# G-Research/ahocorasick_rs

Hardware: NVIDIA H100
Metric: haystack_GB_per_s_scanned_find_matches_as_indexes (higher is better)
Workload: dtype u8

## Files before the change

### ahocorasick_rs_b200/csrc/scan_staged.cuh

```cuda
#pragma once
#include <type_traits>

#include "scan_core.cuh"

namespace acb {

#ifndef ACB_MAX_WARPS
#define ACB_MAX_WARPS 32
#endif
constexpr int kMaxWarps = ACB_MAX_WARPS;
#ifndef ACB_MAX_WARPS2
#define ACB_MAX_WARPS2 22
#endif
constexpr int kMaxWarps2 = ACB_MAX_WARPS2;
constexpr int kChunk = 64;
constexpr int kRow = kChunk;
constexpr int kStageBytes = 32 * kRow;
constexpr int kStageOffset = 256 + 128;
constexpr int kMetaBytes = 32 * 8;

struct FastTab {
    uint32_t cmap;
    uint32_t lo, maxc;
};

__device__ __forceinline__ uint32_t lds_tab(uint32_t addr) {
    uint32_t v;
    asm("ld.shared.u16 %0, [%1];\n" : "=r"(v) : "r"(addr));
    return v;
}
__device__ __forceinline__ uint32_t lds_tab_u8(uint32_t addr) {
    uint32_t v;
    asm("ld.shared.u8 %0, [%1];\n" : "=r"(v) : "r"(addr));
    return v;
}
__device__ __forceinline__ uint4 lds128(uint32_t addr) {
    uint4 v;
    asm volatile("ld.shared.v4.u32 {%0, %1, %2, %3}, [%4];\n" : "=r"(v.x), "=r"(v.y), "=r"(v.z), "=r"(v.w) : "r"(addr));
    return v;
}
__device__ __forceinline__ uint32_t lds8(uint32_t addr) {
    uint32_t v;
    asm volatile("ld.shared.u8 %0, [%1];\n" : "=r"(v) : "r"(addr));
    return v;
}
__device__ __forceinline__ uint32_t lds32(uint32_t addr) {
    uint32_t v;
    asm("ld.shared.u32 %0, [%1];\n" : "=r"(v) : "r"(addr));
    return v;
}
__device__ __forceinline__ uint2 lds64(uint32_t addr) {
    uint2 v;
    asm volatile("ld.shared.v2.u32 {%0, %1}, [%2];\n" : "=r"(v.x), "=r"(v.y) : "r"(addr));
    return v;
}
__device__ __forceinline__ void sts64(uint32_t addr, uint2 v) {
    asm volatile("st.shared.v2.u32 [%0], {%1, %2};\n" ::"r"(addr), "r"(v.x), "r"(v.y) : "memory");
}
__device__ __forceinline__ uint32_t row_unit(uint32_t row, uint32_t j) { return row ^ (j << 4); }
__device__ __forceinline__ uint32_t row_byte(uint32_t row, uint32_t p) { return (row ^ (p & 0x30u)) + (p & 15u); }

constexpr int kColAscii = 2;

template <int COLMODE, bool CLAMP = true>
__device__ __forceinline__ uint32_t fstep(uint32_t s, uint32_t b, const FastTab &f) {
    uint32_t col;
    if (COLMODE == kColRange)
        col = min(b - f.lo, f.maxc);
    else if (COLMODE == kColClass)
        col = lds_tab_u8(f.cmap + b);
    else
        col = CLAMP ? min(b, 127u) : b;
    uint32_t addr;
    asm("mad.lo.u32 %0, %1, 2, %2;\n" : "=r"(addr) : "r"(col), "r"(s));
    return lds_tab(addr);
}

template <uint32_t K>
__device__ __forceinline__ uint32_t fstep_dp(uint32_t s, uint32_t w) {
    uint32_t addr;
    asm("dp4a.u32.u32 %0, %1, %2, %3;\n" : "=r"(addr) : "r"(w), "r"(2u << (8 * K)), "r"(s));
    return lds_tab(addr);
}
__device__ __forceinline__ uint32_t clamp7f(uint32_t w) {
    const uint32_t hi = w & 0x80808080u;
    return (w | (hi - (hi >> 7))) & ~hi;
}

template <int COLMODE, bool CLAMP = true>
__device__ __forceinline__ uint32_t fstep4(uint32_t s, uint32_t w, const FastTab &f) {
    if (COLMODE == kColAscii && !CLAMP) {
        s = fstep_dp<0>(s, w);
        s = fstep_dp<1>(s, w);
        s = fstep_dp<2>(s, w);
        return fstep_dp<3>(s, w);
    }
    s = fstep<COLMODE, CLAMP>(s, __byte_perm(w, 0, 0x4440), f);
    s = fstep<COLMODE, CLAMP>(s, __byte_perm(w, 0, 0x4441), f);
    s = fstep<COLMODE, CLAMP>(s, __byte_perm(w, 0, 0x4442), f);
    s = fstep<COLMODE, CLAMP>(s, __byte_perm(w, 0, 0x4443), f);
    return s;
}

__device__ __forceinline__ uint32_t cont_bytes(uint32_t w) { return __popc(w & ~(w << 1) & 0x80808080u); }

__device__ __forceinline__ void cp_async16(uint32_t dst_smem, const void *src, uint32_t src_bytes) {
    asm volatile("cp.async.cg.shared.global.L2::128B [%0], [%1], 16, %2;\n" ::"r"(dst_smem), "l"(src), "r"(src_bytes) : "memory");
}
__device__ __forceinline__ void cp_async16_last(uint32_t dst_smem, const void *src, uint32_t src_bytes) {
    asm volatile(
        "{\n"
        ".reg .b64 pol;\n"
        "createpolicy.fractional.L2::evict_first.b64 pol, 1.0;\n"
        "cp.async.cg.shared.global.L2::cache_hint.L2::128B [%0], [%1], 16, %2, pol;\n"
        "}\n" ::"r"(dst_smem), "l"(src), "r"(src_bytes)
        : "memory");
}
__device__ __forceinline__ void cp_async_commit() { asm volatile("cp.async.commit_group;\n" ::: "memory"); }
__device__ __forceinline__ void cp_async_wait_all() { asm volatile("cp.async.wait_group 0;\n" ::: "memory"); }

__device__ __forceinline__ void mbar_init(uint32_t bar, uint32_t count) {
    asm volatile("mbarrier.init.shared::cta.b64 [%0], %1;\n" ::"r"(bar), "r"(count) : "memory");
    asm volatile("fence.mbarrier_init.release.cluster;\n" ::: "memory");
}
__device__ __forceinline__ void mbar_expect_tx(uint32_t bar, uint32_t bytes) {
    asm volatile("mbarrier.arrive.expect_tx.shared::cta.b64 _, [%0], %1;\n" ::"r"(bar), "r"(bytes) : "memory");
}
__device__ __forceinline__ void tma_bulk_g2s(uint32_t dst, const void *src, uint32_t bytes, uint32_t bar) {
    asm volatile("cp.async.bulk.shared::cluster.global.mbarrier::complete_tx::bytes [%0], [%1], %2, [%3];\n" ::"r"(dst),
                 "l"(src), "r"(bytes), "r"(bar)
                 : "memory");
}
__device__ __forceinline__ void mbar_wait(uint32_t bar, uint32_t parity) {
    asm volatile(
        "{\n"
        ".reg .pred p;\n"
        "WAIT_%=:\n"
        "mbarrier.try_wait.parity.shared::cta.b64 p, [%0], %1;\n"
        "@p bra DONE_%=;\n"
        "bra WAIT_%=;\n"
        "DONE_%=:\n"
        "}\n" ::"r"(bar),
        "r"(parity)
        : "memory");
}

struct DevHot {
    const uint16_t *table;
    const uint32_t *hot2full;
    const uint16_t *full2hot;
    uint32_t n_rows;
    const uint16_t *table128;
    uint32_t n_rows128;
};

enum PieceKind : uint32_t { kPieceWarm = 0, kPieceHead = 1, kPieceNormal = 2 };
struct LaneSeg {
    int64_t org;
    int64_t seg;
    uint32_t lo_rel, hi_rel;
    uint32_t h;
    uint32_t kind;
    uint32_t spec_state, head_count;
    uint32_t done;
    uint32_t far;
};

template <int MODE, bool CP>
__device__ __forceinline__ void advance_piece(PieceCtx &c, LaneSeg &L, const Batch &B, const Sink &out, const SegOut &seg_out) {
    bool finish_segment = false;
    if (L.kind == kPieceWarm) {
        const uint32_t he_rel = c.limit;
        const uint32_t piece_end = min(L.hi_rel, he_rel);
        if (c.at == L.lo_rel) {
            L.spec_state = c.state;
            L.kind = kPieceHead;
            c.stop = piece_end;
            c.emit_from = 0;
            c.cp_pos = c.at;
            c.cp_cont = 0;
            return;
        }
        L.spec_state = kSpecSkipped;
        L.kind = kPieceHead;
        c.at = piece_end;
        c.stop = piece_end;
        c.emit_from = 0;
        c.state = kRoot;
        c.have = 0;
        c.cp_pos = L.lo_rel;
        c.cp_cont = 0;
    }
    if (L.kind == kPieceHead) L.head_count = c.nemit;
    if (c.stop == c.limit) {
        int64_t h = (int64_t)L.h + 1;
        while (h < B.n_haystacks && __ldg(B.offsets + h + 1) == __ldg(B.offsets + h)) h++;
        const int64_t hi_pos = L.org + L.hi_rel;
        if (h < B.n_haystacks && __ldg(B.offsets + h) < hi_pos) {
            const int64_t hs = __ldg(B.offsets + h), he = __ldg(B.offsets + h + 1);
            L.h = (uint32_t)h;
            L.kind = kPieceNormal;
            c.at = (uint32_t)(hs - L.org);
// ... 53 lines not shown
    const uint32_t cmap_s = hot_s + hot_bytes;
    const uint32_t bar_s = cmap_s + 256;
    const uint32_t h2f_s = cmap_s + kStageOffset;
    const uint32_t stage_all_s = h2f_s + (((H + 1) * 4 + 127u) & ~127u);
    const uint32_t row_entries = COLMODE == kColAscii ? kAsciiCols : im.n_cols;
    const uint32_t row_bytes = row_entries * 2;
    const uint32_t trap_off = H * row_bytes;
    const uint32_t trap = hot_s + trap_off;
    const uint16_t *src_table = COLMODE == kColAscii ? hot_img.table128 : hot_img.table;
    uint8_t *cmap = smem + hot_bytes;
    int64_t *bounds = reinterpret_cast<int64_t *>(smem + hot_bytes + 256 + 16);

    const uint32_t n_entries = (H + 1) * row_entries;
    const uint32_t guard_entries = COLMODE == kColAscii ? kAsciiCols : 0;
    uint32_t *tab32 = reinterpret_cast<uint32_t *>(smem);
    const uint32_t bias2 = hot_s | (hot_s << 16);
    if (H == (COLMODE == kColAscii ? hot_img.n_rows128 : hot_img.n_rows)) {
        const uint32_t bytes = (n_entries * 2 + 15u) & ~15u;
        if (threadIdx.x == 0) {
            mbar_init(bar_s, 1);
            mbar_expect_tx(bar_s, bytes);
            tma_bulk_g2s(hot_s, src_table, bytes, bar_s);
            bounds[0] = __ldg(B.offsets);
            bounds[1] = __ldg(B.offsets + B.n_haystacks);
        }
        for (uint32_t i = threadIdx.x; i < 256; i += blockDim.x) cmap[i] = __ldg(im.colmap + i);
        __syncthreads();
        mbar_wait(bar_s, 0);
        for (uint32_t i = threadIdx.x; i < (n_entries + 1) / 2; i += blockDim.x) tab32[i] += bias2;
    } else {
        const uint32_t n = H * row_entries;
        const uint32_t *src32 = reinterpret_cast<const uint32_t *>(src_table);
        for (uint32_t i = threadIdx.x; i < (n + 1) / 2; i += blockDim.x) {
            const uint32_t v = __ldg(src32 + i);
            tab32[i] = (min(v & 0xffffu, trap_off) | (min(v >> 16, trap_off) << 16)) + bias2;
        }
        __syncthreads();
        uint16_t *h16 = reinterpret_cast<uint16_t *>(smem);
        for (uint32_t i = threadIdx.x; i < row_entries; i += blockDim.x) h16[n + i] = (uint16_t)trap;
        for (uint32_t i = threadIdx.x; i < 256; i += blockDim.x) cmap[i] = __ldg(im.colmap + i);
        if (threadIdx.x == 0) {
            bounds[0] = __ldg(B.offsets);
            bounds[1] = __ldg(B.offsets + B.n_haystacks);
        }
    }
    {
        uint16_t *h16 = reinterpret_cast<uint16_t *>(smem);
        for (uint32_t i = threadIdx.x; i < guard_entries; i += blockDim.x) h16[n_entries + i] = (uint16_t)trap;
        uint32_t *h2f = reinterpret_cast<uint32_t *>(smem + hot_bytes + kStageOffset);
        for (uint32_t i = threadIdx.x; i <= H; i += blockDim.x) h2f[i] = i < H ? __ldg(hot_img.hot2full + i) : kDead;
    }
    __syncthreads();
    if (blockIdx.x == 0 && threadIdx.x == 0) atomicAdd(trap_stats, (unsigned long long)((bounds[1] - bounds[0]) >> 4));

    HotMap hm;
    hm.full2hot = hot_img.full2hot;
    hm.hot_limit = H;
    FastTab ft;
    ft.cmap = cmap_s;
    ft.lo = im.col_lo;
    ft.maxc = im.n_cols - 1;
    auto row_of = [&](uint32_t addr) { return (addr - hot_s) / row_bytes; };
    auto state_of = [&](uint32_t addr) { return lds32(h2f_s + row_of(addr) * 4); };

    const uint32_t lane = threadIdx.x & 31, warp = threadIdx.x >> 5;
    constexpr uint32_t kRows = 32 * V;
    constexpr uint32_t kBufBytes = kRows * kRow;
    constexpr uint32_t kWarpMeta = kRows * 8;
    const uint32_t meta_s = stage_all_s + warp * kWarpMeta;
    const uint32_t stage_s = stage_all_s + (blockDim.x >> 5) * kWarpMeta + warp * 2 * kBufBytes;
    const uintptr_t gbase = reinterpret_cast<uintptr_t>(B.bytes + P.origin);
    const uint32_t cp_dst = stage_s + (lane >> 2) * kRow + (((lane & 3) ^ ((lane >> 3) & 3)) << 4);
    const uint32_t cp_meta = meta_s + (lane >> 2) * 8;
    const uint32_t row_s = stage_s + lane * kRow + (((lane >> 1) & 3) << 4);
    const uint32_t q = P.lane_stride;
    const uint32_t n_tasks = (uint32_t)(((uint64_t)P.n_segments + (uint64_t)kRows * q - 1) / ((uint64_t)kRows * q) * q);

    PieceCtx c_mem[V];
    LaneSeg L_mem[V];
    PieceCtx *c_ptr = c_mem;
    LaneSeg *L_ptr = L_mem;
    asm volatile("" : "+l"(c_ptr), "+l"(L_ptr));

    unsigned int claimed = 0;
    if (lane == 0) claimed = atomicAdd(task_counter, 1u);
    for (;;) {
        const unsigned int task = __shfl_sync(0xffffffffu, claimed, 0);
        if (task >= n_tasks) break;

        uint32_t pos[V], s[V], stop[V], cpd[V];
        uint32_t hi_rel[V], stop_head[V];
        bool done[V], warm[V];
        uint32_t nch_max = 0;
        __syncwarp();
        const int64_t stream_lo = bounds[0], stream_hi = bounds[1];
#pragma unroll
        for (int t = 0; t < V; t++) {
            PieceCtx &c = c_ptr[t];
            LaneSeg &L = L_ptr[t];
            L.seg = (int64_t)(((uint64_t)(task / q) * kRows + (uint32_t)t * 32u + lane) * q + task % q);
            L.done = 1;
            L.spec_state = kNoState;
            L.head_count = 0;
            L.far = 0;
            uint32_t off16 = 0, nchunks = 0;
            pos[t] = 0;
            s[t] = hot_s;
            stop[t] = 0;
            cpd[t] = 0;
            warm[t] = false;
            hi_rel[t] = stop_head[t] = 0;
            const int64_t glo = P.origin + L.seg * (int64_t)P.seg_bytes;
            const int64_t lo = max(glo, stream_lo), hi = min(glo + (int64_t)P.seg_bytes, stream_hi);
            if (L.seg < P.n_segments && lo >= hi) {
                write_summary(seg_out, L.seg, kNoState, kRoot, 0u, 0u, 0u, 0u, false);
            } else if (L.seg < P.n_segments) {
                int64_t h = P.avg_len ? (int64_t)((uint32_t)(lo - stream_lo) / (uint32_t)P.avg_len) : 0;
                if (h >= B.n_haystacks) h = B.n_haystacks - 1;
                int64_t hs = __ldg(B.offsets + h), he = __ldg(B.offsets + h + 1);
                if (!(hs <= lo && lo < he)) {
                    h = find_haystack(B, lo);
                    hs = __ldg(B.offsets + h);
                    he = __ldg(B.offsets + h + 1);
                }
                const bool cont = hs < lo;
                const int64_t w = cont ? max(hs, lo - (int64_t)P.warm) : lo;
                const uintptr_t pw = reinterpret_cast<uintptr_t>(B.bytes + w);
                const uintptr_t a0 = pw & ~uintptr_t(kChunk - 1);
                L.org = w - (int64_t)(pw - a0);
                L.lo_rel = (uint32_t)(lo - L.org);
                L.hi_rel = (uint32_t)(hi - L.org);
                L.h = (uint32_t)h;
                L.kind = cont ? kPieceWarm : kPieceNormal;
                L.done = 0;
                L.far = CP && cont && L.seg - (hs - P.origin) / (int64_t)P.seg_bytes > kContSpan;
                off16 = (uint32_t)((a0 - gbase) >> 4);
                nchunks = (L.hi_rel + kChunk - 1) / kChunk;
                c.base = B.bytes + L.org;
                c.at = (uint32_t)(w - L.org);
                c.limit = (uint32_t)(he - L.org);
                c.stop = cont ? L.lo_rel : min(L.hi_rel, c.limit);
                c.emit_from = cont ? 0xffffffffu : 0u;
                c.state = kRoot;
                c.have = 0;
                c.last_pid = c.last_end = 0;
                c.hay = (uint32_t)h;
                c.hay_delta = (uint32_t)(L.org - hs);
                c.unit = (uint32_t)(2 * L.seg + 1);
                c.nemit = 0;
                c.cp_pos = c.at;
                c.cp_cont = 0;
                warm[t] = cont;
                pos[t] = c.at;
                stop[t] = c.stop;
                hi_rel[t] = L.hi_rel;
                stop_head[t] = min(L.hi_rel, c.limit);
            }
            done[t] = L.done != 0;
            if (done[t]) nchunks = 0;
            nch_max = max(nch_max, nchunks);
            sts64(meta_s + ((uint32_t)t * 32u + lane) * 8, make_uint2(off16, nchunks));
        }
        const uint32_t kmax = __reduce_max_sync(0xffffffffu, nch_max);
        __syncwarp();
        uint2 mrow[4];
        if (V == 1) {
#pragma unroll
            for (int i = 0; i < 4; i++) mrow[i] = lds64(cp_meta + i * 64);
        }

        auto issue = [&](uint32_t k) {
            const uint32_t dst = cp_dst + (k & 1u) * kBufBytes;
#pragma unroll
            for (int i = 0; i < 4 * V; i++) {
                const uint2 m = V == 1 ? mrow[i & 3] : lds64(cp_meta + i * 64);
                const bool live = k < m.y;
                const uint8_t *src = reinterpret_cast<const uint8_t *>(gbase) + (live ? (size_t)(m.x + k * 4 + (lane & 3)) << 4 : 0);
                if (reinterpret_cast<uintptr_t>(src) & 64)
                    cp_async16_last(dst + i * 8 * kRow, src, live ? 16u : 0u);
                else
                    cp_async16(dst + i * 8 * kRow, src, live ? 16u : 0u);
            }
            cp_async_commit();
        };

        auto careful = [&](uint32_t t, uint32_t relk, uint32_t row, bool tail) {
            PieceCtx &c = c_ptr[t];
            LaneSeg &L = L_ptr[t];
            uint32_t S = s[0], POS = pos[0], STOP = stop[0], CPD = cpd[0], HI = hi_rel[0], HEAD = stop_head[0];
            bool DONE = done[0], WARM = warm[0];
#pragma unroll
            for (int u = 1; u < V; u++)
                if (t == (uint32_t)u) {
                    S = s[u];
                    POS = pos[u];
                    STOP = stop[u];
                    CPD = cpd[u];
                    HI = hi_rel[u];
                    HEAD = stop_head[u];
                    DONE = done[u];
                    WARM = warm[u];
                }
            auto leave_fast = [&](uint32_t min_at) {
                c.state = state_of(S);
                c.at = POS;
                if (CP) {
                    c.cp_pos = POS;
                    c.cp_cont = CPD;
                }
                settle<MODE, CP>(c, L, im, B, out, seg_out, hm, min_at);
                DONE = L.done != 0;
                POS = c.at;
                STOP = c.stop;
                WARM = !DONE && L.kind == kPieceWarm;
                if (!DONE) {
                    S = hot_s + (uint32_t)__ldg(hot_img.full2hot + c.state) * row_bytes;
                    if (CP) {
                        cp_catch_up(c, POS);
                        CPD = c.cp_cont;
                    }
                }
            };
            auto piece_end_fast = [&]() -> bool {
                if (WARM) {
                    L.spec_state = state_of(S);
                    L.kind = kPieceHead;
                    STOP = HEAD;
                    c.stop = STOP;
                    c.emit_from = 0;
                    CPD = 0;
                    WARM = false;
                    return true;
                }
                if (STOP == HI) {
                    const int64_t seg = L.seg;
                    const uint32_t nem = c.nemit, spec = L.spec_state, kind = L.kind, hc = L.head_count, far = L.far;
                    write_summary(seg_out, seg, spec, state_of(S), 0u, kind == kPieceHead ? nem : hc, nem, CP ? CPD : 0u, CP && far);
                    L.done = 1;
                    DONE = true;
                    return true;
                }
                return false;
            };
#pragma unroll 1
            for (int j = 0; j < (tail ? 1 : 4); j++) {
                const uint32_t g = relk + j * 16;
                if (!tail) {
                    if (DONE || POS < g || POS >= g + 16) continue;
                    if (POS == g && g + 16 <= STOP) {
                        const uint4 w = lds128(row_unit(row, (uint32_t)j));
                        uint32_t x = fstep4<COLMODE>(S, w.x, ft);
                        x = fstep4<COLMODE>(x, w.y, ft);
                        x = fstep4<COLMODE>(x, w.z, ft);
                        x = fstep4<COLMODE>(x, w.w, ft);
                        if (x != trap) {
                            S = x;
                            POS += 16;
                            if (CP) {
                                if ((w.x | w.y | w.z | w.w) & 0x80808080u)
                                    CPD += cont_bytes(w.x) + cont_bytes(w.y) + cont_bytes(w.z) + cont_bytes(w.w);
                            }
                            continue;
                        }
                    }
                }
                while (!DONE && (tail || (POS >= g && POS < g + 16))) {
                    uint32_t min_at = STOP;
                    if (POS >= STOP) {
                        if (POS == STOP && piece_end_fast()) continue;
                    } else if (!tail) {
                        const uint32_t b = lds8(row_byte(row, POS - relk));
                        const uint32_t x = fstep<COLMODE>(S, b, ft);
                        if (x != trap) {
                            S = x;
                            POS++;
                            if (CP) CPD += (b & 0xC0u) == 0x80u;
                            continue;
                        }
                        atomicAdd(trap_stats + 1, 1ULL);
                        min_at = POS + 1;
                    }
                    leave_fast(min_at);
                }
            }
#pragma unroll
            for (int u = 0; u < V; u++)
                if (t == (uint32_t)u) {
                    s[u] = S;
                    pos[u] = POS;
                    stop[u] = STOP;
                    cpd[u] = CPD;
                    done[u] = DONE;
                    warm[u] = WARM;
                }
        };

        if (kmax)
            issue(0);
        else if (lane == 0)
            claimed = atomicAdd(task_counter, 1u);
        for (uint32_t k = 0; k <= kmax; k++) {
            const bool tail = k == kmax;
            const uint32_t row0 = row_s + (k & 1u) * kBufBytes;
            const uint32_t relk = k * kChunk;
            if (!tail) {
                cp_async_wait_all();
                __syncwarp();
                if (k + 1 < kmax) {
                    issue(k + 1);
                } else if (lane == 0) {
                    claimed = atomicAdd(task_counter, 1u);
                }
                bool clean[V], any_clean = false;
#pragma unroll
                for (int t = 0; t < V; t++) {
                    if (!done[t] && warm[t] && pos[t] == stop[t] && pos[t] == relk) {
                        PieceCtx &c = c_ptr[t];
                        LaneSeg &L = L_ptr[t];
                        L.spec_state = state_of(s[t]);
                        L.kind = kPieceHead;
                        stop[t] = stop_head[t];
                        c.stop = stop[t];
                        c.emit_from = 0;
                        cpd[t] = 0;
                        warm[t] = false;
                    }
                    clean[t] = !done[t] && pos[t] == relk && relk + kChunk <= stop[t];
                    any_clean |= clean[t];
                }
                if (any_clean) {
                    uint32_t x[V], hb[V];
                    uint4 w[V];
#pragma unroll
                    for (int t = 0; t < V; t++) {
                        x[t] = s[t];
                        hb[t] = 0;
                        w[t] = lds128(row0 + t * 32 * kRow);
                    }
#pragma unroll
                    for (int j = 0; j < 4; j++) {
                        uint4 wn[V];
#pragma unroll
                        for (int t = 0; t < V; t++) {
                            wn[t] = w[t];
                            if (j < 3) wn[t] = lds128(row_unit(row0 + t * 32 * kRow, (uint32_t)j + 1));
                        }
#pragma unroll
                        for (int t = 0; t < V; t++) {
                            if (CP || COLMODE == kColAscii) hb[t] |= w[t].x | w[t].y | w[t].z | w[t].w;
                            if (COLMODE == kColAscii) {
                                if ((w[t].x | w[t].y | w[t].z | w[t].w) & 0x80808080u) {
                                    w[t].x = clamp7f(w[t].x);
                                    w[t].y = clamp7f(w[t].y);
                                    w[t].z = clamp7f(w[t].z);
                                    w[t].w = clamp7f(w[t].w);
                                }
                            }
                        }
#pragma unroll
                        for (int t = 0; t < V; t++) x[t] = fstep4<COLMODE, false>(x[t], w[t].x, ft);
#pragma unroll
                        for (int t = 0; t < V; t++) x[t] = fstep4<COLMODE, false>(x[t], w[t].y, ft);
#pragma unroll
                        for (int t = 0; t < V; t++) x[t] = fstep4<COLMODE, false>(x[t], w[t].z, ft);
#pragma unroll
                        for (int t = 0; t < V; t++) x[t] = fstep4<COLMODE, false>(x[t], w[t].w, ft);
#pragma unroll
                        for (int t = 0; t < V; t++) w[t] = wn[t];
                    }
#pragma unroll
                    for (int t = 0; t < V; t++) {
                        const bool high = (hb[t] & 0x80808080u) != 0;
                        if (clean[t] && x[t] != trap) {
                            s[t] = x[t];
                            pos[t] += kChunk;
                            if (CP && high) {
#pragma unroll
                                for (int j = 0; j < 4; j++) {
                                    const uint4 v = lds128(row_unit(row0 + t * 32 * kRow, (uint32_t)j));
                                    cpd[t] += cont_bytes(v.x) + cont_bytes(v.y) + cont_bytes(v.z) + cont_bytes(v.w);
                                }
                            }
                        }
                    }
                }
            }
            uint32_t need = 0;
#pragma unroll
            for (int t = 0; t < V; t++) need |= (!done[t] && (tail || pos[t] < relk + kChunk)) ? (1u << t) : 0u;
            if (need) {
#pragma unroll 1
                for (uint32_t t = 0; t < (uint32_t)V; t++)
                    if (need & (1u << t)) careful(t, relk, row0 + t * 32 * kRow, tail);
            }
        }
    }
}

}
```

### profiles/microbench/stage_copy.cu

```cuda
#include <cstdint>
#include <cstdio>
#include <cuda_runtime.h>

template <int PF, bool EVF = false>
__device__ __forceinline__ void cp_async16(uint32_t dst, const void *src, uint64_t pol = 0) {
    if (EVF) {
        asm volatile("cp.async.cg.shared.global.L2::cache_hint.L2::128B [%0], [%1], 16, %2;\n" ::"r"(dst), "l"(src), "l"(pol) : "memory");
        return;
    }
    if (PF == 0) asm volatile("cp.async.cg.shared.global [%0], [%1], 16;\n" ::"r"(dst), "l"(src) : "memory");
    if (PF == 1) asm volatile("cp.async.cg.shared.global.L2::128B [%0], [%1], 16;\n" ::"r"(dst), "l"(src) : "memory");
    if (PF == 2) asm volatile("cp.async.cg.shared.global.L2::256B [%0], [%1], 16;\n" ::"r"(dst), "l"(src) : "memory");
}
__device__ __forceinline__ void prefetch_l2(const void *src, uint32_t bytes) {
    asm volatile("cp.async.bulk.prefetch.L2.global [%0], %1;\n" ::"l"(src), "r"(bytes) : "memory");
}
__device__ __forceinline__ void cp_commit() { asm volatile("cp.async.commit_group;\n" ::: "memory"); }
template <int N> __device__ __forceinline__ void cp_wait() { asm volatile("cp.async.wait_group %0;\n" ::"n"(N) : "memory"); }

constexpr uint32_t kQ = 4, kSeg = 1024, kBuf = 32 * 64, kRec = 28;

struct Lever {
    bool model;
    int pfc, pfd;
    bool next;
    bool evf;
    int warps;
};

template <int STAGES, int PF, bool MODEL, bool EVF>
__global__ void __launch_bounds__(1024, 1) stage(const uint8_t *data, uint32_t n_rows, uint32_t spin, int pfc, int pfd, bool next_pf,
                                                 unsigned int *counter, unsigned long long *stats, uint32_t *sink, uint4 *summaries) {
    extern __shared__ __align__(128) uint8_t smem[];
    const uint32_t lane = threadIdx.x & 31, warp = threadIdx.x >> 5;
    const uint32_t stage = (uint32_t)__cvta_generic_to_shared(smem) + warp * STAGES * kBuf;
    const uint32_t n_tasks = n_rows / 32;
    uint32_t acc = 0;
    unsigned long long waited = 0;
    uint64_t pol = 0;
    if (EVF) asm volatile("createpolicy.fractional.L2::evict_first.b64 %0, 1.0;\n" : "=l"(pol));
    uint32_t rec[kRec];
    uint32_t *rp = rec;
    asm volatile("" : "+l"(rp));
    const long long t_start = clock64();
    unsigned int claimed = 0;
    if (MODEL && lane == 0) claimed = atomicAdd(counter, 1u);
    for (;;) {
        if (!MODEL && lane == 0) claimed = atomicAdd(counter, 1u);
        const unsigned int task = __shfl_sync(0xffffffffu, claimed, 0);
        if (task >= n_tasks) break;
        const uint64_t seg0 = (uint64_t)(task / kQ) * 32 * kQ + task % kQ;
        const bool warm = MODEL && task % kQ != 0;
        const uint32_t kmax = kSeg / 64 + (warm ? 1 : 0);
        const int64_t first = warm ? -64 : 0;
        if (MODEL) {
#pragma unroll
            for (int i = 0; i < (int)kRec; i++) rp[i] = (uint32_t)(seg0 + lane) * (i + 1);
        }
        const uint8_t *mine = data + (int64_t)((seg0 + (uint64_t)lane * kQ) * kSeg) + first;
        auto issue = [&](uint32_t k) {
            if (k < kmax) {
                const uint32_t buf = stage + (k % STAGES) * kBuf;
#pragma unroll
                for (int i = 0; i < 4; i++) {
                    const uint32_t r = i * 8 + (lane >> 2);
                    const uint8_t *src = data + (int64_t)((seg0 + (uint64_t)r * kQ) * kSeg) + first + k * 64 + (lane & 3) * 16;
                    const uint32_t dst = buf + r * 64 + (((lane & 3) ^ ((r >> 1) & 3)) << 4);
                    if (EVF && (reinterpret_cast<uintptr_t>(src) & 64))
                        cp_async16<PF, true>(dst, src, pol);
                    else
                        cp_async16<PF>(dst, src);
                }
            }
            cp_commit();
        };
        const uint32_t k_claim = next_pf ? kmax - 2 : kmax - 1;
        for (uint32_t k = 0; k + 1 < STAGES; k++) issue(k);
        for (uint32_t k = 0; k < kmax; k++) {
            const long long w0 = clock64();
            cp_wait<STAGES - 2>();
            __syncwarp();
            waited += (unsigned long long)(clock64() - w0);
            issue(k + STAGES - 1);
            if (MODEL && k == k_claim && lane == 0) claimed = atomicAdd(counter, 1u);
            if (pfc && k % pfc == 0 && k + pfd < kmax) {
                const uint32_t n = min((uint32_t)pfc, kmax - (k + pfd));
                prefetch_l2(mine + (k + pfd) * 64, n * 64);
            }
            if (next_pf && k == kmax - 1) {
                const unsigned int nt = __shfl_sync(0xffffffffu, claimed, 0);
                if (nt < n_tasks) {
                    const uint64_t ns = ((uint64_t)(nt / kQ) * 32 * kQ + nt % kQ) + (uint64_t)lane * kQ;
                    const int64_t nf = nt % kQ != 0 ? -64 : 0;
                    prefetch_l2(data + (int64_t)(ns * kSeg) + nf, max(pfc, 4) * 64);
                }
            }
            uint32_t v;
            asm volatile("ld.shared.u32 %0, [%1];\n" : "=r"(v) : "r"(stage + (k % STAGES) * kBuf + lane * 64));
            acc += v;
            const long long t0 = clock64();
            while (clock64() - t0 < spin) {}
        }
        if (MODEL) {
            uint32_t x = 0;
#pragma unroll
            for (int i = 0; i < (int)kRec; i++) x += rp[i];
            summaries[2 * (seg0 + (uint64_t)lane * kQ)] = make_uint4(x, acc, 0, 0);
            summaries[2 * (seg0 + (uint64_t)lane * kQ) + 1] = make_uint4(0, 0, x, 1);
        }
        cp_wait<0>();
    }
    if (lane == 0) {
        atomicAdd(stats, waited);
        atomicAdd(stats + 1, (unsigned long long)(clock64() - t_start));
    }
    if (acc == 0x12345678u) sink[0] = acc;
}

template <int STAGES, int PF, bool MODEL, bool EVF>
void run(const char *name, const uint8_t *d, uint32_t rows, uint32_t spin, double clock_ghz, int sms, Lever lv, uint4 *summ) {
    unsigned int *ctr; unsigned long long *st; uint32_t *sink;
    cudaMalloc(&ctr, 4); cudaMalloc(&st, 16); cudaMalloc(&sink, 4);
    const size_t smem = (size_t)lv.warps * STAGES * kBuf;
    cudaFuncSetAttribute(stage<STAGES, PF, MODEL, EVF>, cudaFuncAttributeMaxDynamicSharedMemorySize, (int)smem);
    float best = 1e9, sum = 0; unsigned long long h[2] = {0, 0};
    const int iters = 20;
    for (int it = 0; it < iters + 2; it++) {
        cudaMemset(ctr, 0, 4); cudaMemset(st, 0, 16);
        cudaEvent_t e0, e1; cudaEventCreate(&e0); cudaEventCreate(&e1);
        cudaEventRecord(e0);
        stage<STAGES, PF, MODEL, EVF><<<sms, lv.warps * 32, smem>>>(d, rows, spin, lv.pfc, lv.pfd, lv.next, ctr, st, sink, summ);
        cudaEventRecord(e1); cudaEventSynchronize(e1);
        float ms; cudaEventElapsedTime(&ms, e0, e1);
        if (it >= 2) sum += ms;
        if (ms < best) { best = ms; cudaMemcpy(h, st, 16, cudaMemcpyDeviceToHost); }
        cudaEventDestroy(e0); cudaEventDestroy(e1);
    }
    const double chunks = MODEL ? 16.75 : 16.0;
    const double spin_ms = (double)rows / 32 / (sms * lv.warps) * chunks * spin / clock_ghz / 1e6;
    printf("%-34s spin %5u cyc: best %.4f ms, mean %.4f (spin alone %.4f), %6.1f GB/s, wait %.1f %% of warp time  (%s)\n", name, spin,
           best, sum / iters, spin_ms, (double)rows * kSeg / best / 1e6, 100.0 * h[0] / (double)h[1], cudaGetErrorString(cudaGetLastError()));
    cudaFree(ctr); cudaFree(st); cudaFree(sink);
}

int main() {
    cudaDeviceProp p; cudaGetDeviceProperties(&p, 0);
    int khz = 0; cudaDeviceGetAttribute(&khz, cudaDevAttrClockRate, 0);
    const double ghz = khz / 1e6;
    const uint32_t rows = 400000;
    const int sms = p.multiProcessorCount;
    uint8_t *base; cudaMalloc(&base, (size_t)rows * kSeg + 256); cudaMemset(base, 1, (size_t)rows * kSeg + 256);
    const uint8_t *d = base + 128;
    uint4 *summ; cudaMalloc(&summ, (size_t)rows * 32);
    printf("%s, %d SMs, max SM clock %.3f GHz\n", p.name, sms, ghz);
    for (double us : {2.4, 2.8}) {
        const uint32_t spin = (uint32_t)(us * 1e3 * ghz);
        run<2, 1, false, false>("copies only, L2::128B", d, rows, spin, ghz, sms, {false, 0, 0, false, false, 32}, summ);
        run<2, 1, true, false>("model, L2::128B", d, rows, spin, ghz, sms, {true, 0, 0, false, false, 32}, summ);
        char name[64];
        for (int pfc : {2, 4, 8})
            for (int pfd : {1, 2, 4, 8}) {
                if (pfd < pfc / 2) continue;
                snprintf(name, sizeof name, "(a) R=%d D=%d", pfc * 64, pfd);
                run<2, 1, true, false>(name, d, rows, spin, ghz, sms, {true, pfc, pfd, false, false, 32}, summ);
            }
        run<2, 1, true, false>("(b) next task, 256 B", d, rows, spin, ghz, sms, {true, 0, 0, true, false, 32}, summ);
        run<2, 1, true, false>("(a)+(b) R=256 D=4", d, rows, spin, ghz, sms, {true, 4, 4, true, false, 32}, summ);
        run<2, 1, true, true>("(c) evict_first", d, rows, spin, ghz, sms, {true, 0, 0, false, true, 32}, summ);
        run<2, 1, true, true>("(a)+(b)+(c) R=256 D=4", d, rows, spin, ghz, sms, {true, 4, 4, true, true, 32}, summ);
        for (int w : {16, 24}) {
            snprintf(name, sizeof name, "(d) %d warps", w);
            run<2, 1, true, false>(name, d, rows, spin, ghz, sms, {true, 0, 0, false, false, w}, summ);
            snprintf(name, sizeof name, "(d) %d warps + (a)+(b) R=512 D=8", w);
            run<2, 1, true, false>(name, d, rows, spin, ghz, sms, {true, 8, 8, true, false, w}, summ);
        }
    }
    cudaFree(base); cudaFree(summ);
    return 0;
}
```

Measured before the change: 1512.

## Defer per-lane segment records and overlap first two stage copies

Segment setup is factored into an open_segment helper. Full per-lane PieceCtx/LaneSeg records are now built lazily, only when a lane leaves the fast path, and are otherwise reconstructed from the shared-memory metadata. Warm-up handling moves into a packed flags word that also carries a speculative state, and only the 16-byte pieces actually needed for a warm chunk are copied. The first two chunks are issued back to back with wait_group 1, so chunk 1's copy overlaps chunk 0's processing. This cuts register and local-memory traffic and start-of-task latency, at the cost of more complex state bookkeeping and recomputing segment geometry on slow-path exits.

```diff
diff --git a/ahocorasick_rs_b200/csrc/scan_staged.cuh b/ahocorasick_rs_b200/csrc/scan_staged.cuh
--- a/ahocorasick_rs_b200/csrc/scan_staged.cuh
+++ b/ahocorasick_rs_b200/csrc/scan_staged.cuh
@@ -18,6 +18,7 @@
 constexpr int kStageBytes = 32 * kRow;
 constexpr int kStageOffset = 256 + 128;
 constexpr int kMetaBytes = 32 * 8;
+constexpr uint32_t kMetaWarmChunk = 0x80000000u;
 
 struct FastTab {
     uint32_t cmap;
@@ -116,8 +117,12 @@
         "}\n" ::"r"(dst_smem), "l"(src), "r"(src_bytes)
         : "memory");
 }
+__device__ __forceinline__ void cp_async16_warm(uint32_t dst_smem, const void *src, uint32_t src_bytes) {
+    asm volatile("cp.async.cg.shared.global [%0], [%1], 16, %2;\n" ::"r"(dst_smem), "l"(src), "r"(src_bytes) : "memory");
+}
 __device__ __forceinline__ void cp_async_commit() { asm volatile("cp.async.commit_group;\n" ::: "memory"); }
 __device__ __forceinline__ void cp_async_wait_all() { asm volatile("cp.async.wait_group 0;\n" ::: "memory"); }
+__device__ __forceinline__ void cp_async_wait_one() { asm volatile("cp.async.wait_group 1;\n" ::: "memory"); }
 
 __device__ __forceinline__ void mbar_init(uint32_t bar, uint32_t count) {
     asm volatile("mbarrier.init.shared::cta.b64 [%0], %1;\n" ::"r"(bar), "r"(count) : "memory");
@@ -337,6 +342,58 @@
     LaneSeg *L_ptr = L_mem;
     asm volatile("" : "+l"(c_ptr), "+l"(L_ptr));
 
+    auto open_segment = [&](int64_t seg, PieceCtx &c, LaneSeg &L) -> bool {
+        L.seg = seg;
+        L.done = 1;
+        L.spec_state = kNoState;
+        L.head_count = 0;
+        L.far = 0;
+        const int64_t stream_lo = bounds[0], stream_hi = bounds[1];
+        const int64_t glo = P.origin + seg * (int64_t)P.seg_bytes;
+        const int64_t lo = max(glo, stream_lo), hi = min(glo + (int64_t)P.seg_bytes, stream_hi);
+        if (seg >= P.n_segments) return false;
+        if (lo >= hi) return true;
+        int64_t h = P.avg_len ? (int64_t)((uint32_t)(lo - stream_lo) / (uint32_t)P.avg_len) : 0;
+        if (h >= B.n_haystacks) h = B.n_haystacks - 1;
+        int64_t hs = __ldg(B.offsets + h), he = __ldg(B.offsets + h + 1);
+        if (!(hs <= lo && lo < he)) {
+            h = find_haystack(B, lo);
+            hs = __ldg(B.offsets + h);
+            he = __ldg(B.offsets + h + 1);
+        }
+        const bool cont = hs < lo;
+        const int64_t w = cont ? max(hs, lo - (int64_t)P.warm) : lo;
+        const uintptr_t pw = reinterpret_cast<uintptr_t>(B.bytes + w);
+        const uintptr_t a0 = pw & ~uintptr_t(kChunk - 1);
+        L.org = w - (int64_t)(pw - a0);
+        L.lo_rel = (uint32_t)(lo - L.org);
+        L.hi_rel = (uint32_t)(hi - L.org);
+        L.h = (uint32_t)h;
+        L.kind = cont ? kPieceWarm : kPieceNormal;
+        L.done = 0;
+        L.far = CP && cont && seg - (hs - P.origin) / (int64_t)P.seg_bytes > kContSpan;
+        c.base = B.bytes + L.org;
+        c.at = (uint32_t)(w - L.org);
+        c.limit = (uint32_t)(he - L.org);
+        c.stop = cont ? L.lo_rel : min(L.hi_rel, c.limit);
+        c.emit_from = cont ? 0xffffffffu : 0u;
+        c.state = kRoot;
+        c.have = 0;
+        c.last_pid = c.last_end = 0;
+        c.hay = (uint32_t)h;
+        c.hay_delta = (uint32_t)(L.org - hs);
+        c.unit = (uint32_t)(2 * seg + 1);
+        c.nemit = 0;
+        c.cp_pos = c.at;
+        c.cp_cont = 0;
+        return false;
+    };
+    constexpr uint32_t kFlWarm = 1, kFlSpec = 2, kFlRec = 4;
+    auto seg_of = [&](uint32_t t, bool cont) {
+        const uint64_t rel = (uint64_t)(lds64(meta_s + (t * 32u + lane) * 8).x & ~3u) << 4;
+        return (int64_t)(rel / P.seg_bytes) + (cont ? 1 : 0);
+    };
+
     unsigned int claimed = 0;
     if (lane == 0) claimed = atomicAdd(task_counter, 1u);
     for (;;) {
@@ -345,67 +402,30 @@
 
         uint32_t pos[V], s[V], stop[V], cpd[V];
         uint32_t hi_rel[V], stop_head[V];
-        bool done[V], warm[V];
+        uint32_t fl[V];
+        bool done[V];
         uint32_t nch_max = 0;
         __syncwarp();
-        const int64_t stream_lo = bounds[0], stream_hi = bounds[1];
 #pragma unroll
         for (int t = 0; t < V; t++) {
-            PieceCtx &c = c_ptr[t];
-            LaneSeg &L = L_ptr[t];
-            L.seg = (int64_t)(((uint64_t)(task / q) * kRows + (uint32_t)t * 32u + lane) * q + task % q);
-            L.done = 1;
-            L.spec_state = kNoState;
-            L.head_count = 0;
-            L.far = 0;
+            PieceCtx c;
+            LaneSeg L;
             uint32_t off16 = 0, nchunks = 0;
             pos[t] = 0;
             s[t] = hot_s;
             stop[t] = 0;
             cpd[t] = 0;
-            warm[t] = false;
+            fl[t] = 0;
             hi_rel[t] = stop_head[t] = 0;
-            const int64_t glo = P.origin + L.seg * (int64_t)P.seg_bytes;
-            const int64_t lo = max(glo, stream_lo), hi = min(glo + (int64_t)P.seg_bytes, stream_hi);
-            if (L.seg < P.n_segments && lo >= hi) {
-                write_summary(seg_out, L.seg, kNoState, kRoot, 0u, 0u, 0u, 0u, false);
-            } else if (L.seg < P.n_segments) {
-                int64_t h = P.avg_len ? (int64_t)((uint32_t)(lo - stream_lo) / (uint32_t)P.avg_len) : 0;
-                if (h >= B.n_haystacks) h = B.n_haystacks - 1;
-                int64_t hs = __ldg(B.offsets + h), he = __ldg(B.offsets + h + 1);
-                if (!(hs <= lo && lo < he)) {
-                    h = find_haystack(B, lo);
-                    hs = __ldg(B.offsets + h);
-                    he = __ldg(B.offsets + h + 1);
-                }
-                const bool cont = hs < lo;
-                const int64_t w = cont ? max(hs, lo - (int64_t)P.warm) : lo;
-                const uintptr_t pw = reinterpret_cast<uintptr_t>(B.bytes + w);
-                const uintptr_t a0 = pw & ~uintptr_t(kChunk - 1);
-                L.org = w - (int64_t)(pw - a0);
-                L.lo_rel = (uint32_t)(lo - L.org);
-                L.hi_rel = (uint32_t)(hi - L.org);
-                L.h = (uint32_t)h;
-                L.kind = cont ? kPieceWarm : kPieceNormal;
-                L.done = 0;
-                L.far = CP && cont && L.seg - (hs - P.origin) / (int64_t)P.seg_bytes > kContSpan;
-                off16 = (uint32_t)((a0 - gbase) >> 4);
+            const int64_t seg = (int64_t)(((uint64_t)(task / q) * kRows + (uint32_t)t * 32u + lane) * q + task % q);
+            if (open_segment(seg, c, L)) write_summary(seg_out, seg, kNoState, kRoot, 0u, 0u, 0u, 0u, false);
+            uint32_t meta_x = 0, meta_y = 0;
+            if (!L.done) {
+                off16 = (uint32_t)((reinterpret_cast<uintptr_t>(c.base) - gbase) >> 4);
                 nchunks = (L.hi_rel + kChunk - 1) / kChunk;
-                c.base = B.bytes + L.org;
-                c.at = (uint32_t)(w - L.org);
-                c.limit = (uint32_t)(he - L.org);
-                c.stop = cont ? L.lo_rel : min(L.hi_rel, c.limit);
-                c.emit_from = cont ? 0xffffffffu : 0u;
-                c.state = kRoot;
-                c.have = 0;
-                c.last_pid = c.last_end = 0;
-                c.hay = (uint32_t)h;
-                c.hay_delta = (uint32_t)(L.org - hs);
-                c.unit = (uint32_t)(2 * L.seg + 1);
-                c.nemit = 0;
-                c.cp_pos = c.at;
-                c.cp_cont = 0;
-                warm[t] = cont;
+                meta_x = off16 | (c.at >> 4);
+                meta_y = nchunks | (L.lo_rel == kChunk ? kMetaWarmChunk : 0u);
+                fl[t] = L.kind == kPieceWarm ? kFlWarm : 0u;
                 pos[t] = c.at;
                 stop[t] = c.stop;
                 hi_rel[t] = L.hi_rel;
@@ -414,7 +434,7 @@
             done[t] = L.done != 0;
             if (done[t]) nchunks = 0;
             nch_max = max(nch_max, nchunks);
-            sts64(meta_s + ((uint32_t)t * 32u + lane) * 8, make_uint2(off16, nchunks));
+            sts64(meta_s + ((uint32_t)t * 32u + lane) * 8, make_uint2(meta_x, meta_y));
         }
         const uint32_t kmax = __reduce_max_sync(0xffffffffu, nch_max);
         __syncwarp();
@@ -429,9 +449,11 @@
 #pragma unroll
             for (int i = 0; i < 4 * V; i++) {
                 const uint2 m = V == 1 ? mrow[i & 3] : lds64(cp_meta + i * 64);
-                const bool live = k < m.y;
-                const uint8_t *src = reinterpret_cast<const uint8_t *>(gbase) + (live ? (size_t)(m.x + k * 4 + (lane & 3)) << 4 : 0);
-                if (reinterpret_cast<uintptr_t>(src) & 64)
+                const bool live = k < (m.y & ~kMetaWarmChunk) && (k != 0 || (lane & 3) >= (m.x & 3u));
+                const uint8_t *src = reinterpret_cast<const uint8_t *>(gbase) + (live ? (size_t)((m.x & ~3u) + k * 4 + (lane & 3)) << 4 : 0);
+                if (k == 0 && (m.y & kMetaWarmChunk))
+                    cp_async16_warm(dst + i * 8 * kRow, src, live ? 16u : 0u);
+                else if (reinterpret_cast<uintptr_t>(src) & 64)
                     cp_async16_last(dst + i * 8 * kRow, src, live ? 16u : 0u);
                 else
                     cp_async16(dst + i * 8 * kRow, src, live ? 16u : 0u);
@@ -442,8 +464,8 @@
         auto careful = [&](uint32_t t, uint32_t relk, uint32_t row, bool tail) {
             PieceCtx &c = c_ptr[t];
             LaneSeg &L = L_ptr[t];
-            uint32_t S = s[0], POS = pos[0], STOP = stop[0], CPD = cpd[0], HI = hi_rel[0], HEAD = stop_head[0];
-            bool DONE = done[0], WARM = warm[0];
+            uint32_t S = s[0], POS = pos[0], STOP = stop[0], CPD = cpd[0], HI = hi_rel[0], HEAD = stop_head[0], FL = fl[0];
+            bool DONE = done[0];
 #pragma unroll
             for (int u = 1; u < V; u++)
                 if (t == (uint32_t)u) {
@@ -453,10 +475,19 @@
                     CPD = cpd[u];
                     HI = hi_rel[u];
                     HEAD = stop_head[u];
+                    FL = fl[u];
                     DONE = done[u];
-                    WARM = warm[u];
                 }
             auto leave_fast = [&](uint32_t min_at) {
+                if (!(FL & kFlRec)) {
+                    open_segment(seg_of(t, FL & (kFlWarm | kFlSpec)), c, L);
+                    if (FL & kFlSpec) {
+                        L.spec_state = state_of(FL >> 16);
+                        L.kind = kPieceHead;
+                        c.stop = STOP;
+                        c.emit_from = 0;
+                    }
+                }
                 c.state = state_of(S);
                 c.at = POS;
                 if (CP) {
@@ -467,7 +498,7 @@
                 DONE = L.done != 0;
                 POS = c.at;
                 STOP = c.stop;
-                WARM = !DONE && L.kind == kPieceWarm;
+                FL = kFlRec | (!DONE && L.kind == kPieceWarm ? kFlWarm : 0u);
                 if (!DONE) {
                     S = hot_s + (uint32_t)__ldg(hot_img.full2hot + c.state) * row_bytes;
                     if (CP) {
@@ -477,21 +508,30 @@
                 }
             };
             auto piece_end_fast = [&]() -> bool {
-                if (WARM) {
-                    L.spec_state = state_of(S);
-                    L.kind = kPieceHead;
+                if (FL & kFlWarm) {
                     STOP = HEAD;
-                    c.stop = STOP;
-                    c.emit_from = 0;
                     CPD = 0;
-                    WARM = false;
+                    if (FL & kFlRec) {
+                        L.spec_state = state_of(S);
+                        L.kind = kPieceHead;
+                        c.stop = STOP;
+                        c.emit_from = 0;
+                        FL = kFlRec;
+                    } else {
+                        FL = kFlSpec | (S << 16);
+                    }
                     return true;
                 }
                 if (STOP == HI) {
-                    const int64_t seg = L.seg;
-                    const uint32_t nem = c.nemit, spec = L.spec_state, kind = L.kind, hc = L.head_count, far = L.far;
-                    write_summary(seg_out, seg, spec, state_of(S), 0u, kind == kPieceHead ? nem : hc, nem, CP ? CPD : 0u, CP && far);
-                    L.done = 1;
+                    if (FL & kFlRec) {
+                        const int64_t seg = L.seg;
+                        const uint32_t nem = c.nemit, spec = L.spec_state, kind = L.kind, hc = L.head_count, far = L.far;
+                        write_summary(seg_out, seg, spec, state_of(S), 0u, kind == kPieceHead ? nem : hc, nem, CP ? CPD : 0u, CP && far);
+                        L.done = 1;
+                    } else {
+                        const uint32_t spec = FL & kFlSpec ? state_of(FL >> 16) : kNoState;
+                        write_summary(seg_out, seg_of(t, FL & kFlSpec), spec, state_of(S), 0u, 0u, 0u, CP ? CPD : 0u, false);
+                    }
                     DONE = true;
                     return true;
                 }
@@ -546,39 +586,48 @@
                     stop[u] = STOP;
                     cpd[u] = CPD;
                     done[u] = DONE;
-                    warm[u] = WARM;
+                    fl[u] = FL;
                 }
         };
 
-        if (kmax)
+        if (kmax) {
             issue(0);
-        else if (lane == 0)
+            if (kmax > 1) issue(1);
+        } else if (lane == 0) {
             claimed = atomicAdd(task_counter, 1u);
+        }
         for (uint32_t k = 0; k <= kmax; k++) {
             const bool tail = k == kmax;
             const uint32_t row0 = row_s + (k & 1u) * kBufBytes;
             const uint32_t relk = k * kChunk;
             if (!tail) {
-                cp_async_wait_all();
+                if (k == 0 && kmax > 1)
+                    cp_async_wait_one();
+                else
+                    cp_async_wait_all();
                 __syncwarp();
                 if (k + 1 < kmax) {
-                    issue(k + 1);
+                    if (k > 0) issue(k + 1);
                 } else if (lane == 0) {
                     claimed = atomicAdd(task_counter, 1u);
                 }
                 bool clean[V], any_clean = false;
 #pragma unroll
                 for (int t = 0; t < V; t++) {
-                    if (!done[t] && warm[t] && pos[t] == stop[t] && pos[t] == relk) {
-                        PieceCtx &c = c_ptr[t];
-                        LaneSeg &L = L_ptr[t];
-                        L.spec_state = state_of(s[t]);
-                        L.kind = kPieceHead;
+                    if (!done[t] && (fl[t] & kFlWarm) && pos[t] == stop[t] && pos[t] == relk) {
                         stop[t] = stop_head[t];
-                        c.stop = stop[t];
-                        c.emit_from = 0;
                         cpd[t] = 0;
-                        warm[t] = false;
+                        if (fl[t] & kFlRec) {
+                            PieceCtx &c = c_ptr[t];
+                            LaneSeg &L = L_ptr[t];
+                            L.spec_state = state_of(s[t]);
+                            L.kind = kPieceHead;
+                            c.stop = stop[t];
+                            c.emit_from = 0;
+                            fl[t] = kFlRec;
+                        } else {
+                            fl[t] = kFlSpec | (s[t] << 16);
+                        }
                     }
                     clean[t] = !done[t] && pos[t] == relk && relk + kChunk <= stop[t];
                     any_clean |= clean[t];
diff --git a/profiles/microbench/stage_copy.cu b/profiles/microbench/stage_copy.cu
--- a/profiles/microbench/stage_copy.cu
+++ b/profiles/microbench/stage_copy.cu
@@ -17,23 +17,32 @@
 }
 __device__ __forceinline__ void cp_commit() { asm volatile("cp.async.commit_group;\n" ::: "memory"); }
 template <int N> __device__ __forceinline__ void cp_wait() { asm volatile("cp.async.wait_group %0;\n" ::"n"(N) : "memory"); }
+__device__ __forceinline__ void spin_for(uint32_t cycles) {
+    const long long t0 = clock64();
+    while (clock64() - t0 < cycles) {}
+}
 
 constexpr uint32_t kQ = 4, kSeg = 1024, kBuf = 32 * 64, kRec = 28;
+constexpr uint32_t kWarmArea = 32 * 16;
 
 struct Lever {
-    bool model;
+    bool warm, rec, summ, claim;
+    bool warm16, early0;
     int pfc, pfd;
     bool next;
     bool evf;
     int warps;
 };
-
-template <int STAGES, int PF, bool MODEL, bool EVF>
-__global__ void __launch_bounds__(1024, 1) stage(const uint8_t *data, uint32_t n_rows, uint32_t spin, int pfc, int pfd, bool next_pf,
-                                                 unsigned int *counter, unsigned long long *stats, uint32_t *sink, uint4 *summaries) {
+constexpr Lever kModel = {true, true, true, true, false, false, 0, 0, false, false, 32};
+constexpr Lever kCopies = {false, false, false, false, false, false, 0, 0, false, false, 32};
+
+template <int STAGES, int PF, bool EVF>
+__global__ void __launch_bounds__(1024, 1) stage(const uint8_t *data, uint32_t n_rows, uint32_t spin, Lever lv, unsigned int *counter,
+                                                 unsigned long long *stats, uint32_t *sink, uint4 *summaries) {
     extern __shared__ __align__(128) uint8_t smem[];
     const uint32_t lane = threadIdx.x & 31, warp = threadIdx.x >> 5;
     const uint32_t stage = (uint32_t)__cvta_generic_to_shared(smem) + warp * STAGES * kBuf;
+    const uint32_t warm_s = (uint32_t)__cvta_generic_to_shared(smem) + (blockDim.x >> 5) * STAGES * kBuf + warp * kWarmArea;
     const uint32_t n_tasks = n_rows / 32;
     uint32_t acc = 0;
     unsigned long long waited = 0;
@@ -43,73 +52,118 @@
     uint32_t *rp = rec;
     asm volatile("" : "+l"(rp));
     const long long t_start = clock64();
+    struct Task {
+        uint64_t seg0;
+        bool warm;
+        uint32_t kmax;
+        int64_t first;
+    };
+    auto geometry = [&](unsigned int t) {
+        Task g;
+        g.seg0 = (uint64_t)(t / kQ) * 32 * kQ + t % kQ;
+        g.warm = lv.warm && t % kQ != 0;
+        const bool chunk = g.warm && !lv.warm16;
+        g.kmax = kSeg / 64 + (chunk ? 1 : 0);
+        g.first = chunk ? -64 : 0;
+        return g;
+    };
+    auto issue = [&](const Task &g, uint32_t k, uint32_t par) {
+        if (k < g.kmax) {
+            const uint32_t buf = stage + ((k + par) % STAGES) * kBuf;
+#pragma unroll
+            for (int i = 0; i < 4; i++) {
+                const uint32_t r = i * 8 + (lane >> 2);
+                const uint8_t *src = data + (int64_t)((g.seg0 + (uint64_t)r * kQ) * kSeg) + g.first + k * 64 + (lane & 3) * 16;
+                const uint32_t dst = buf + r * 64 + (((lane & 3) ^ ((r >> 1) & 3)) << 4);
+                if (EVF && (reinterpret_cast<uintptr_t>(src) & 64))
+                    cp_async16<PF, true>(dst, src, pol);
+                else
+                    cp_async16<PF>(dst, src);
+            }
+            if (k == 0 && g.warm && lv.warm16)
+                cp_async16<PF>(warm_s + lane * 16, data + (int64_t)((g.seg0 + (uint64_t)lane * kQ) * kSeg) - 16);
+        }
+        cp_commit();
+    };
     unsigned int claimed = 0;
-    if (MODEL && lane == 0) claimed = atomicAdd(counter, 1u);
+    uint32_t par = 0;
+    bool pre = false;
+    if (lv.claim && lane == 0) claimed = atomicAdd(counter, 1u);
     for (;;) {
-        if (!MODEL && lane == 0) claimed = atomicAdd(counter, 1u);
+        if (!lv.claim && lane == 0) claimed = atomicAdd(counter, 1u);
         const unsigned int task = __shfl_sync(0xffffffffu, claimed, 0);
         if (task >= n_tasks) break;
-        const uint64_t seg0 = (uint64_t)(task / kQ) * 32 * kQ + task % kQ;
-        const bool warm = MODEL && task % kQ != 0;
-        const uint32_t kmax = kSeg / 64 + (warm ? 1 : 0);
-        const int64_t first = warm ? -64 : 0;
-        if (MODEL) {
+        const Task g = geometry(task);
+        const uint64_t seg0 = g.seg0;
+        const uint32_t kmax = g.kmax;
+        if (lv.rec) {
 #pragma unroll
             for (int i = 0; i < (int)kRec; i++) rp[i] = (uint32_t)(seg0 + lane) * (i + 1);
         }
-        const uint8_t *mine = data + (int64_t)((seg0 + (uint64_t)lane * kQ) * kSeg) + first;
-        auto issue = [&](uint32_t k) {
-            if (k < kmax) {
-                const uint32_t buf = stage + (k % STAGES) * kBuf;
-#pragma unroll
-                for (int i = 0; i < 4; i++) {
-                    const uint32_t r = i * 8 + (lane >> 2);
-                    const uint8_t *src = data + (int64_t)((seg0 + (uint64_t)r * kQ) * kSeg) + first + k * 64 + (lane & 3) * 16;
-                    const uint32_t dst = buf + r * 64 + (((lane & 3) ^ ((r >> 1) & 3)) << 4);
-                    if (EVF && (reinterpret_cast<uintptr_t>(src) & 64))
-                        cp_async16<PF, true>(dst, src, pol);
-                    else
-                        cp_async16<PF>(dst, src);
-                }
-            }
-            cp_commit();
-        };
-        const uint32_t k_claim = next_pf ? kmax - 2 : kmax - 1;
-        for (uint32_t k = 0; k + 1 < STAGES; k++) issue(k);
+        const uint8_t *mine = data + (int64_t)((seg0 + (uint64_t)lane * kQ) * kSeg) + g.first;
+        const uint32_t k_claim = lv.next ? kmax - 2 : kmax - 1;
+        if (!pre)
+            for (uint32_t k = 0; k + 1 < STAGES; k++) issue(g, k, par);
+        pre = false;
         for (uint32_t k = 0; k < kmax; k++) {
             const long long w0 = clock64();
             cp_wait<STAGES - 2>();
             __syncwarp();
             waited += (unsigned long long)(clock64() - w0);
-            issue(k + STAGES - 1);
-            if (MODEL && k == k_claim && lane == 0) claimed = atomicAdd(counter, 1u);
-            if (pfc && k % pfc == 0 && k + pfd < kmax) {
-                const uint32_t n = min((uint32_t)pfc, kmax - (k + pfd));
-                prefetch_l2(mine + (k + pfd) * 64, n * 64);
-            }
-            if (next_pf && k == kmax - 1) {
+            if (lv.early0 && k + 1 == kmax) {
+                if (lane == 0) claimed = atomicAdd(counter, 1u);
+            } else {
+                issue(g, k + STAGES - 1, par);
+                if (lv.claim && k == k_claim && lane == 0) claimed = atomicAdd(counter, 1u);
+            }
+            if (lv.pfc && k % lv.pfc == 0 && k + lv.pfd < kmax) {
+                const uint32_t n = min((uint32_t)lv.pfc, kmax - (k + lv.pfd));
+                prefetch_l2(mine + (k + lv.pfd) * 64, n * 64);
+            }
+            if (lv.next && k == kmax - 1) {
                 const unsigned int nt = __shfl_sync(0xffffffffu, claimed, 0);
                 if (nt < n_tasks) {
                     const uint64_t ns = ((uint64_t)(nt / kQ) * 32 * kQ + nt % kQ) + (uint64_t)lane * kQ;
                     const int64_t nf = nt % kQ != 0 ? -64 : 0;
-                    prefetch_l2(data + (int64_t)(ns * kSeg) + nf, max(pfc, 4) * 64);
+                    prefetch_l2(data + (int64_t)(ns * kSeg) + nf, max(lv.pfc, 4) * 64);
                 }
             }
             uint32_t v;
-            asm volatile("ld.shared.u32 %0, [%1];\n" : "=r"(v) : "r"(stage + (k % STAGES) * kBuf + lane * 64));
+            if (k == 0 && g.warm && lv.warm16) {
+                asm volatile("ld.shared.u32 %0, [%1];\n" : "=r"(v) : "r"(warm_s + lane * 16));
+                acc += v;
+                spin_for(spin / 4);
+            }
+            asm volatile("ld.shared.u32 %0, [%1];\n" : "=r"(v) : "r"(stage + ((k + par) % STAGES) * kBuf + lane * 64));
             acc += v;
-            const long long t0 = clock64();
-            while (clock64() - t0 < spin) {}
-        }
-        if (MODEL) {
-            uint32_t x = 0;
+            spin_for(k == 0 && g.first ? spin / 4 : spin);
+        }
+        const uint32_t next_par = (kmax + par) % STAGES;
+        if (lv.early0) {
+            const unsigned int nt = __shfl_sync(0xffffffffu, claimed, 0);
+            if (nt < n_tasks) {
+                issue(geometry(nt), 0, next_par);
+                pre = true;
+            }
+        }
+        uint32_t x = 0;
+        if (lv.rec) {
 #pragma unroll
             for (int i = 0; i < (int)kRec; i++) x += rp[i];
+        }
+        if (lv.summ) {
             summaries[2 * (seg0 + (uint64_t)lane * kQ)] = make_uint4(x, acc, 0, 0);
             summaries[2 * (seg0 + (uint64_t)lane * kQ) + 1] = make_uint4(0, 0, x, 1);
-        }
-        cp_wait<0>();
-    }
+        } else {
+            acc += x;
+        }
+        if (lv.early0) {
+            par = next_par;
+        } else {
+            cp_wait<0>();
+        }
+    }
+    cp_wait<0>();
     if (lane == 0) {
         atomicAdd(stats, waited);
         atomicAdd(stats + 1, (unsigned long long)(clock64() - t_start));
@@ -117,28 +171,28 @@
     if (acc == 0x12345678u) sink[0] = acc;
 }
 
-template <int STAGES, int PF, bool MODEL, bool EVF>
+template <int STAGES, int PF, bool EVF>
 void run(const char *name, const uint8_t *d, uint32_t rows, uint32_t spin, double clock_ghz, int sms, Lever lv, uint4 *summ) {
     unsigned int *ctr; unsigned long long *st; uint32_t *sink;
     cudaMalloc(&ctr, 4); cudaMalloc(&st, 16); cudaMalloc(&sink, 4);
-    const size_t smem = (size_t)lv.warps * STAGES * kBuf;
-    cudaFuncSetAttribute(stage<STAGES, PF, MODEL, EVF>, cudaFuncAttributeMaxDynamicSharedMemorySize, (int)smem);
+    const size_t smem = (size_t)lv.warps * (STAGES * kBuf + kWarmArea);
+    cudaFuncSetAttribute(stage<STAGES, PF, EVF>, cudaFuncAttributeMaxDynamicSharedMemorySize, (int)smem);
     float best = 1e9, sum = 0; unsigned long long h[2] = {0, 0};
     const int iters = 20;
     for (int it = 0; it < iters + 2; it++) {
         cudaMemset(ctr, 0, 4); cudaMemset(st, 0, 16);
         cudaEvent_t e0, e1; cudaEventCreate(&e0); cudaEventCreate(&e1);
         cudaEventRecord(e0);
-        stage<STAGES, PF, MODEL, EVF><<<sms, lv.warps * 32, smem>>>(d, rows, spin, lv.pfc, lv.pfd, lv.next, ctr, st, sink, summ);
+        stage<STAGES, PF, EVF><<<sms, lv.warps * 32, smem>>>(d, rows, spin, lv, ctr, st, sink, summ);
         cudaEventRecord(e1); cudaEventSynchronize(e1);
         float ms; cudaEventElapsedTime(&ms, e0, e1);
         if (it >= 2) sum += ms;
         if (ms < best) { best = ms; cudaMemcpy(h, st, 16, cudaMemcpyDeviceToHost); }
         cudaEventDestroy(e0); cudaEventDestroy(e1);
     }
-    const double chunks = MODEL ? 16.75 : 16.0;
+    const double chunks = lv.warm ? 16.0 + 0.75 / 4 : 16.0;
     const double spin_ms = (double)rows / 32 / (sms * lv.warps) * chunks * spin / clock_ghz / 1e6;
-    printf("%-34s spin %5u cyc: best %.4f ms, mean %.4f (spin alone %.4f), %6.1f GB/s, wait %.1f %% of warp time  (%s)\n", name, spin,
+    printf("%-40s spin %5u cyc: best %.4f ms, mean %.4f (spin alone %.4f), %6.1f GB/s, wait %.1f %% of warp time  (%s)\n", name, spin,
            best, sum / iters, spin_ms, (double)rows * kSeg / best / 1e6, 100.0 * h[0] / (double)h[1], cudaGetErrorString(cudaGetLastError()));
     cudaFree(ctr); cudaFree(st); cudaFree(sink);
 }
@@ -155,24 +209,44 @@
     printf("%s, %d SMs, max SM clock %.3f GHz\n", p.name, sms, ghz);
     for (double us : {2.4, 2.8}) {
         const uint32_t spin = (uint32_t)(us * 1e3 * ghz);
-        run<2, 1, false, false>("copies only, L2::128B", d, rows, spin, ghz, sms, {false, 0, 0, false, false, 32}, summ);
-        run<2, 1, true, false>("model, L2::128B", d, rows, spin, ghz, sms, {true, 0, 0, false, false, 32}, summ);
+        Lever lv;
+        run<2, 1, false>("copies only, L2::128B", d, rows, spin, ghz, sms, kCopies, summ);
+        run<2, 1, false>("model, L2::128B", d, rows, spin, ghz, sms, kModel, summ);
+        run<2, 1, true>("model + evict_first", d, rows, spin, ghz, sms, {true, true, true, true, false, false, 0, 0, false, true, 32}, summ);
+        lv = kModel; lv.evf = true; lv.warm = false;
+        run<2, 1, true>("  without the warm-up chunk", d, rows, spin, ghz, sms, lv, summ);
+        lv = kModel; lv.evf = true; lv.rec = false;
+        run<2, 1, true>("  without the local record", d, rows, spin, ghz, sms, lv, summ);
+        lv = kModel; lv.evf = true; lv.summ = false;
+        run<2, 1, true>("  without the summaries", d, rows, spin, ghz, sms, lv, summ);
+        lv = kModel; lv.evf = true; lv.claim = false;
+        run<2, 1, true>("  claim at the task's top", d, rows, spin, ghz, sms, lv, summ);
+        lv = kModel; lv.evf = true; lv.warm = lv.rec = lv.summ = false;
+        run<2, 1, true>("  none of them (claim kept)", d, rows, spin, ghz, sms, lv, summ);
+        lv = kModel; lv.evf = true; lv.rec = false;
+        run<2, 1, true>("  (1) record off", d, rows, spin, ghz, sms, lv, summ);
+        lv = kModel; lv.evf = true; lv.warm16 = true;
+        run<2, 1, true>("  (2) warm-up with chunk 0", d, rows, spin, ghz, sms, lv, summ);
+        lv = kModel; lv.evf = true; lv.early0 = true;
+        run<2, 1, true>("  (3) next chunk 0 before the tail", d, rows, spin, ghz, sms, lv, summ);
+        lv = kModel; lv.evf = true; lv.rec = false; lv.warm16 = true;
+        run<2, 1, true>("  (1)+(2)", d, rows, spin, ghz, sms, lv, summ);
+        lv = kModel; lv.evf = true; lv.warm16 = true; lv.early0 = true;
+        run<2, 1, true>("  (2)+(3)", d, rows, spin, ghz, sms, lv, summ);
+        lv = kModel; lv.evf = true; lv.rec = false; lv.warm16 = true; lv.early0 = true;
+        run<2, 1, true>("  (1)+(2)+(3)", d, rows, spin, ghz, sms, lv, summ);
+        if (us != 2.4) continue;
         char name[64];
         for (int pfc : {2, 4, 8})
             for (int pfd : {1, 2, 4, 8}) {
                 if (pfd < pfc / 2) continue;
                 snprintf(name, sizeof name, "(a) R=%d D=%d", pfc * 64, pfd);
-                run<2, 1, true, false>(name, d, rows, spin, ghz, sms, {true, pfc, pfd, false, false, 32}, summ);
-            }
-        run<2, 1, true, false>("(b) next task, 256 B", d, rows, spin, ghz, sms, {true, 0, 0, true, false, 32}, summ);
-        run<2, 1, true, false>("(a)+(b) R=256 D=4", d, rows, spin, ghz, sms, {true, 4, 4, true, false, 32}, summ);
-        run<2, 1, true, true>("(c) evict_first", d, rows, spin, ghz, sms, {true, 0, 0, false, true, 32}, summ);
-        run<2, 1, true, true>("(a)+(b)+(c) R=256 D=4", d, rows, spin, ghz, sms, {true, 4, 4, true, true, 32}, summ);
+                run<2, 1, false>(name, d, rows, spin, ghz, sms, {true, true, true, true, false, false, pfc, pfd, false, false, 32}, summ);
+            }
+        run<2, 1, false>("(b) next task, 256 B", d, rows, spin, ghz, sms, {true, true, true, true, false, false, 0, 0, true, false, 32}, summ);
         for (int w : {16, 24}) {
             snprintf(name, sizeof name, "(d) %d warps", w);
-            run<2, 1, true, false>(name, d, rows, spin, ghz, sms, {true, 0, 0, false, false, w}, summ);
-            snprintf(name, sizeof name, "(d) %d warps + (a)+(b) R=512 D=8", w);
-            run<2, 1, true, false>(name, d, rows, spin, ghz, sms, {true, 8, 8, true, false, w}, summ);
+            run<2, 1, false>(name, d, rows, spin, ghz, sms, {true, true, true, true, false, false, 0, 0, false, false, w}, summ);
         }
     }
     cudaFree(base); cudaFree(summ);
```

Measured after the change: 1549, median of 6. 1.02x the previous value.
